# Dsouza10082/nats-llm-studio

Measured on AMD Instinct MI355X. Metric: output tokens/sec + p50 NATS req-reply RTT, Llama-3-8B Q4_K chat_model, higher is better.
Workload: dtype fp16; 1 GPU; model=llama-3-8b Q4_K_M, global_batch=512, seq_len=128, parallelism=dp1, concurrency_per_replica=512, hipgraph=True, device=cuda

## Files before the change

### csrc/kernels/qgemv.hip

```cpp
#include "qgemm_impl.h"
#include "qgemm_dma.h"

using namespace nls_gemv;

namespace nls_hgemm {
int launch_dense(int wm, int bn, int waves, int nst, const SegList& sl, int ntiles, int ks, float* ws,
                 const GemvArgs& a, hipStream_t st);
}
namespace nls_hg10 {
int launch_dense10(int bn, const SegList& sl, int ntiles, int ks, float* ws, const GemvArgs& a, hipStream_t st);
}
namespace nls_q9 {
int launch_q9(int kset, int waves, int rt, const SegList& sl, int ntiles, int ks, float* ws, const GemvArgs& a,
              hipStream_t st, int bm);
}


extern "C" {

struct NlsSeg {
  const void* w;
  const int* xmap;
  const int* ymap;
  const int* mcount;
  int type, rows, K, ycol;
};

struct NlsFuse {
  const float* xf; long ldxf; const float* nw; float eps;
  const int* pos; const int* slot; const float* cs; const float* bias;
  void* q_out; long ldq; void* kc; void* vc; int Hq, Hkv, D, pad0;
  void* hout; long ldh; const float* onw; int* cnt;
  float* ssq_out; const float* ssq_in; int ldss, nss_in;
  const int* sel; int sel_slots, sel_base, pad1;
  const void* wr; int E, topk, renorm, rcap;
  float* rlogits; float* topw; int* counts; int* xrows; int* yrows; int* rsel;
  const void* tab; int tab_n, tab_cap;
};

struct NlsPlan {
  int kset;
  int tile_rows;
  int tiles;
  int cols;
  int slab_width;
  int mapped_splitk;
  int reduce;
  int pad;
  long ws_floats;
};

}

namespace {

inline bool mapped(const NlsSeg& s) { return s.xmap || s.ymap || s.mcount; }

bool norm_in_ok(const NlsFuse& f, int M, int mode) {
  if (f.xf && (M > 16 || !f.nw || (mode != 0 && !(mode == 1 && f.ssq_in)))) return false;
  if (f.ssq_in && (!f.xf || f.nss_in < 1 || f.nss_in > f.ldss)) return false;
  return true;
}

bool norm_producer_ok(const NlsFuse& f, const NlsSeg* segs, int nseg, int M, int epi, const void* argmax, int waves,
                      int rt, int mode) {
  if (!f.ssq_out) return true;
  const int ncols = ((M + 15) / 16) * 16;
  return !(mode != 0 || epi != EPI_ADD_F32 || nseg != 1 || mapped(segs[0]) || argmax || f.onw || M > 32 ||
           (waves * 64) % ncols || f.ldss < (segs[0].rows + 16 * rt - 1) / (16 * rt));
}

bool rope_ok(const NlsFuse& f, const NlsSeg* segs, int nseg, int epi, const void* argmax, int mode, int ks) {
  if (epi != EPI_ROPE) return true;
  if (!(mode == 0 || ((mode == 4 || mode == 5 || mode == 10) && ks <= 1)) || argmax || !f.pos || !f.slot || !f.cs ||
      !f.q_out || !f.kc || !f.vc || f.D < 2 || f.D % 2 || f.Hq < 1 || f.Hkv < 1)
    return false;
  int c = 0;
  for (int i = 0; i < nseg; ++i) {
    if (mapped(segs[i]) || segs[i].rows % 16 || segs[i].ycol != c) return false;
    c += segs[i].rows;
  }
  return c == (f.Hq + 2 * f.Hkv) * f.D;
}

bool add_norm_ok(const NlsFuse& f, const NlsSeg* segs, int nseg, int M, int epi, const void* argmax, int mode) {
  if (f.onw && (mode != 0 || epi != EPI_ADD_F32 || nseg != 1 || segs[0].ycol || mapped(segs[0]) || !f.cnt ||
                !f.hout || segs[0].rows % 4 || argmax))
    return false;
  if (f.wr && (!f.onw || M > 4 || f.E < 1 || f.E > 64 || f.topk < 1 || f.topk > f.E || f.topk > 8 || !f.rlogits ||
               !f.topw || !f.counts || !f.xrows || !f.yrows || segs[0].rows % 4))
    return false;
  return true;
}

bool selected_ok(const NlsFuse& f, const NlsSeg* segs, int nseg, const void* argmax, int mode) {
  if (!f.sel) return true;
  if (mode != 0 || f.sel_slots < 1 || f.sel_slots > 256 || argmax) return false;
  for (int i = 1; i < nseg; ++i)
    if (segs[i].rows != segs[0].rows || segs[i].K != segs[0].K) return false;
  return true;
}

bool table_ok(const NlsFuse& f, const NlsSeg* segs, int nseg, int epi, const void* argmax, int mode, int ks) {
  if (!f.tab) return true;
  return !(nseg != 1 || mode < 0 || mode > 2 || ks > 1 || f.tab_n < 1 || f.tab_cap < 1 || !segs[0].mcount ||
           argmax || f.xf || f.onw || f.ssq_out || epi == EPI_ROPE || epi == EPI_SLABS);
}

bool mode_shape_ok(const NlsFuse& f, const NlsSeg* segs, int nseg, long ldx, long ldy, int M, int epi, int waves,
                   int rt, int mode) {
  if (waves != 4 && waves != 8 && !(waves == 16 && mode >= 4) && !(waves == 7 && mode == 1 && rt == 1 && M == 1))
    return false;
  if (mode < 0 || mode > 10 || mode == 7 || mode == 8 || (mode == 6 && (waves != 8 || rt != 2))) return false;
  const bool unaligned_y = (epi == EPI_F32 || epi == EPI_ADD_F32 || epi == EPI_ACT) && ldy % 4;
  if (mode == 10) {
    if (waves != 8 || (rt != 1 && rt != 2) || f.xf || f.onw || ldx % 8 || unaligned_y) return false;
    for (int i = 0; i < nseg; ++i)
      if (segs[i].type != QT_F16 || mapped(segs[i]) || segs[i].ycol % 4) return false;
  } else if (mode == 9) {
    if (!((waves == 4 && rt == 2) || (waves == 8 && (rt == 2 || rt == 1))) || f.xf || f.onw || epi == EPI_ROPE ||
        ldx % 8 || unaligned_y)
      return false;
    for (int i = 0; i < nseg; ++i)
      if (mapped(segs[i]) || segs[i].ycol % 4) return false;
  } else if (mode >= 4) {
    if ((waves != 8 && waves != 16) || (rt != 2 && rt != 4) || f.xf || f.onw || (epi == EPI_ROPE && mode == 6))
      return false;
    for (int i = 0; i < nseg; ++i)
      if (segs[i].type != QT_F16) return false;
  } else if (mode == 3) {
    if (waves != 4 || (rt != 4 && rt != 6 && rt != 8 && rt != 16)) return false;
    for (int i = 0; i < nseg; ++i)
      if (segs[i].type == QT_Q8_0) return false;
  } else if (mode == 2 ? (waves != 8 || (rt != 1 && rt != 2 && rt != 4)) : (rt != 1 && rt != 2)) {
    return false;
  }
  return !(M > 64 && mode == 0);
}

int type_set(const NlsSeg* segs, int nseg) {
  bool q4k = false, q5k = false, q6k = false, q8 = false, q51 = false, iq4 = false, flt = false, bad = false;
  for (int i = 0; i < nseg; ++i) {
    const int t = segs[i].type;
    if (t == QT_Q4_K) q4k = true;
    else if (t == QT_Q5_K) q5k = true;
    else if (t == QT_Q8_0) q8 = true;
    else if (t == QT_Q51) q51 = true;
    else if (t == QT_IQ4) iq4 = true;
    else if (t == QT_F16 || t == QT_BF16 || t == QT_F32) flt = true;
    else if (t == QT_Q6_K) q6k = true;
    else bad = true;
  }
  if (bad || (flt && (q4k || q5k || q6k || q8 || q51 || iq4)) || (q4k && (q5k || q8 || q51 || iq4)) ||
      (q51 && (q5k || iq4)))
    return -1;
  return flt ? 2 : (q51 ? 3 : (iq4 ? 4 : (q4k ? 0 : ((q5k || q8) ? 1 : 0))));
}

inline int mtiles(int M) { return M > 64 ? 8 : (M + 15) / 16; }
inline int mblocks(int M) { return M > 64 ? (M + 127) / 128 : 1; }

int plan(const NlsSeg* segs, int nseg, const void* x, long ldx, void* y, long ldy, int M, float alpha, int epi,
         void* argmax, int waves, int rt, int mode, int ks, const void* ws, long ws_floats, const NlsFuse& f,
         NlsPlan& p, SegList& sl, GemvArgs& a) {
  if (nseg < 1 || nseg > 8 || M < 1) return -1;
  if (!mode_shape_ok(f, segs, nseg, ldx, ldy, M, epi, waves, rt, mode) || !norm_in_ok(f, M, mode) ||
      !norm_producer_ok(f, segs, nseg, M, epi, argmax, waves, rt, mode) ||
      !rope_ok(f, segs, nseg, epi, argmax, mode, ks) || !add_norm_ok(f, segs, nseg, M, epi, argmax, mode) ||
      !selected_ok(f, segs, nseg, argmax, mode) || !table_ok(f, segs, nseg, epi, argmax, mode, ks))
    return -1;
  if (mode != 0 && ks > 1 && !ws) return -1;
  if (epi == EPI_SLABS && (mode == 0 || ks < 2)) return -1;
  bool mks = (mode >= 1 && mode <= 5) && ks > 1 && epi == EPI_F32 && !argmax;
  for (int i = 0; i < nseg && mks; ++i)
    mks = segs[i].ymap && segs[i].ycol == 0 && segs[i].rows == segs[0].rows;
  sl = SegList{};
  int tiles = 0, cols = 0;
  const int tile_rows = mode == 10 ? 256 / rt : mode == 9 ? 16 * waves * rt
                        : (mode == 5 ? 256 : (mode >= 2 ? 128 : (mode == 1 ? waves : 1) * rt * 16));
  for (int i = 0; i < nseg; ++i) {
    if (segs[i].K % 256 || segs[i].rows < 1) return -1;
    if (epi == EPI_SWIGLU && segs[i].rows % 16) return -1;
    if (mapped(segs[i]) && mode != 0 &&
        (!(mode >= 1 && mode <= 5) || argmax || epi == EPI_SLABS || (ks > 1 && !mks)))
      return -1;
    sl.s[i] = Seg{(const uint8_t*)segs[i].w, segs[i].xmap, segs[i].ymap, segs[i].mcount, segs[i].type, segs[i].rows,
                  segs[i].K,  tiles, segs[i].ycol,  cols};
    tiles += (segs[i].rows + tile_rows - 1) / tile_rows;
    cols += segs[i].rows;
  }
  sl.nseg = nseg;
  if (f.tab) tiles *= f.tab_n;
  const int sel_tiles = (segs[0].rows + tile_rows - 1) / tile_rows;
  if (f.sel) tiles = f.sel_slots * sel_tiles;
  const int kset = type_set(segs, nseg);
  if (kset < 0) return -1;
  if (mode >= 2 && mode <= 3 && kset >= 2) return -1;
  if (mode == 9 && kset == 2) return -1;
  const int nks = mode != 0 && ks > 1 ? ks : 1;
  if (mode == 0 && f.xf && !staged_lds_a(sl, waves, rt, mtiles(M), M)) return -1;
  if (mode == 1 && (f.xf || waves == 7) && !staged_lds_b(sl, mtiles(M), M, nks, mblocks(M), f.xf)) return -1;
  p = NlsPlan{};
  p.kset = kset;
  p.tile_rows = tile_rows;
  p.tiles = tiles;
  p.cols = cols;
  p.slab_width = mks ? segs[0].rows : cols;
  p.mapped_splitk = mks;
  p.reduce = nks > 1 && epi != EPI_SLABS;
  p.ws_floats = nks > 1 ? (long)nks * M * p.slab_width : 0;
  if (ws_floats < p.ws_floats) return -1;
  a = GemvArgs{(const act_t*)(f.xf ? (const void*)f.xf : x), ldx, y, ldy, M, epi, alpha,  p.slab_width,
               (unsigned long long*)argmax,  0,  M,
               f.xf, f.ldxf, f.nw, f.eps,
               f.pos, f.slot, f.cs, f.bias, (__bf16*)f.q_out, f.ldq, (__bf16*)f.kc, (__bf16*)f.vc, f.Hq, f.Hkv, f.D,
               (act_t*)f.hout, f.ldh, f.onw, f.cnt,
               f.ssq_out, f.ssq_in, f.ldss, f.nss_in,
               f.sel, sel_tiles, f.sel_base,  0,
               (const act_t*)f.wr, f.E, f.topk, f.renorm, f.rcap,
               f.rlogits, f.topw, f.counts, f.xrows, f.yrows, f.rsel,
               (const uint8_t* const*)f.tab, f.tab_n, f.tab_cap};
  return 0;
}

int run(const NlsPlan& p, const SegList& sl, const GemvArgs& a, int waves, int rt, int mode, int ks, float* ws,
        hipStream_t st) {
  const int M = a.M, mt = mtiles(M);
  auto launch = p.kset == 0 ? launch_k0
                            : p.kset == 1 ? launch_k1 : p.kset == 2 ? launch_k2 : p.kset == 3 ? launch_k3 : launch_k4;
  if (mode == 0) return launch(0, waves, rt, mt, sl, p.tiles, 1, nullptr, a, st, 1);
  if (ks < 1) ks = 1;
  int rc;
  if (mode == 10)
    rc = nls_hg10::launch_dense10(256 / rt, sl, p.tiles, ks, ws, a, st);
  else if (mode == 9)
    rc = nls_q9::launch_q9(p.kset, waves, rt, sl, p.tiles, ks, ws, a, st, 256);
  else if (mode >= 4)
    rc = nls_hgemm::launch_dense(rt, mode == 5 ? 256 : 128, waves, mode == 6 ? 2 : 3, sl, p.tiles, ks, ws, a, st);
  else if (mode == 3)
    rc = (p.kset == 0 ? nls_dma::launch_dma_k0 : nls_dma::launch_dma_k1)(rt, sl, p.tiles, ks, ws, a, st);
  else if (mode == 2)
    rc = (p.kset == 0 ? nls_gemm::launch_lds_k0 : nls_gemm::launch_lds_k1)(rt, sl, p.tiles, ks, ws, a, st);
  else
    rc = launch(1, waves, rt, mt, sl, p.tiles, ks, ws, a, st, mblocks(M));
  if (rc || !p.reduce) return rc;
  RedList rl{};
  if (p.mapped_splitk) {
    rl.s[0] = RedSeg{0, p.slab_width, 0, 0};
    rl.nseg = 1;
  } else {
    for (int i = 0; i < sl.nseg; ++i) rl.s[i] = RedSeg{sl.s[i].tile_begin_col, sl.s[i].rows, sl.s[i].ycol, 0};
    rl.nseg = sl.nseg;
  }
  const int nout = a.epi == EPI_SWIGLU ? p.slab_width / 2 : p.slab_width;
  dim3 grid((nout + 255) / 256, M);
  hipLaunchKernelGGL(splitk_reduce_kernel, grid, dim3(256), 0, st, (const float*)ws, ks, M, p.slab_width, rl, a);
  return (int)hipGetLastError();
}

const NlsFuse kNoFuse{};

}

extern "C" {

int nls_qgemv(const NlsSeg* segs, int nseg, const void* x, long ldx, void* y, long ldy, int M, float alpha, int epi,
              void* argmax, int waves, int rt, int mode, int ks, void* ws, long ws_floats, void* stream,
              const NlsFuse* fz) {
  NlsPlan p;
  SegList sl;
  GemvArgs a;
  if (plan(segs, nseg, x, ldx, y, ldy, M, alpha, epi, argmax, waves, rt, mode, ks, ws, ws_floats, fz ? *fz : kNoFuse,
           p, sl, a))
    return -1;
  return run(p, sl, a, waves, rt, mode, ks, (float*)ws, (hipStream_t)stream);
}

int nls_qgemv_plan(const NlsSeg* segs, int nseg, const void* x, long ldx, void* y, long ldy, int M, float alpha,
                   int epi, void* argmax, int waves, int rt, int mode, int ks, void* ws, long ws_floats, void* stream,
                   const NlsFuse* fz, NlsPlan* out) {
  SegList sl;
  GemvArgs a;
  (void)stream;
  return plan(segs, nseg, x, ldx, y, ldy, M, alpha, epi, argmax, waves, rt, mode, ks, ws, ws_floats,
              fz ? *fz : kNoFuse, *out, sl, a);
}

int nls_fuse_size() { return (int)sizeof(NlsFuse); }
int nls_plan_size() { return (int)sizeof(NlsPlan); }

}
```

### nats_llm_studio_amd/ops/__init__.py

```python
from __future__ import annotations

import ctypes
import math
import warnings
from dataclasses import dataclass
from typing import List, Optional, Sequence

import numpy as np
import torch

from ..gguf.constants import GGMLType, GGML_BLOCK
from ..gguf.quants import dequantize
from . import _lib
from . import transcode

EPI = {"f32": 0, "act": 1, "add": 2, "swiglu": 3, "slabs": 4, "argmax": 5, "rope": 6}
import os as _os
ADDNORM_MAX_M = int(_os.environ.get("NLS_ADDNORM", "0"))
DENSE_MIN_M = int(_os.environ.get("NLS_DENSE_GEMM_M", "128"))
MOE_GEMV = tuple(int(v) for v in _os.environ.get("NLS_MOE_GEMV", "0,4,2,1").split(","))
ACT_DTYPE = torch.float16


def _stream_ptr(t: torch.Tensor) -> int:
# ... 72 lines not shown
class QWeight:

    def __init__(self, raw: np.ndarray, ggml_type: int, rows: int, K: int, device, name: str = "",
                 layout: str = "tiled"):
        self.gtype = int(ggml_type)
        self.type = int(ggml_type)
        self.rows = int(rows)
        self.K = int(K)
        self.name = name
        self.layout = layout
        self.device = torch.device(device)
        if K % 256:
            raise ValueError(f"{name}: K={K} is not a multiple of 256")
        with warnings.catch_warnings():
            warnings.simplefilter("ignore", UserWarning)
            if GGMLType(ggml_type) in transcode.TRANSCODED:
                t = torch.from_numpy(np.ascontiguousarray(np.asarray(raw).view(np.uint8).reshape(-1)))
                t = t.to(self.device) if self.device.type != "cpu" else t
                t, self.type = transcode.device_form(t, ggml_type, rows, K, layout)
                if layout == "rows":
                    t = torch.from_numpy(np.ascontiguousarray(to_device_layout(t.cpu().numpy(), self.type, rows, K)))
                    self.data = t.to(self.device) if self.device.type != "cpu" else t.clone()
                elif self.type in (transcode.QT_Q51, transcode.QT_IQ4):
                    self.data = t
                else:
                    self.data = tile_layout(t, self.type, rows, K)
            elif layout == "rows":
                t = torch.from_numpy(np.ascontiguousarray(to_device_layout(raw, ggml_type, rows, K)))
                self.data = t.to(self.device) if self.device.type != "cpu" else t.clone()
            else:
                t = torch.from_numpy(np.ascontiguousarray(np.asarray(raw).view(np.uint8).reshape(-1)))
                t = t.to(self.device) if self.device.type != "cpu" else t
                self.data = tile_layout(t, ggml_type, rows, K)
        self._raw = np.ascontiguousarray(raw).view(np.uint8).reshape(-1) if self.device.type == "cpu" else None
        self._dense = None
        self.d16: Optional[torch.Tensor] = None

    def to_f16(self) -> "QWeight":
        if self.device.type == "cpu" or self.type == int(GGMLType.F16):
            return self
        w = QWeight.__new__(QWeight)
        w.__dict__.update(self.__dict__)
        w.type = int(GGMLType.F16)
        w.data = tile_layout(self.dense(torch.float16).contiguous().view(torch.uint8).reshape(-1), GGMLType.F16,
                             self.rows, self.K)
        w.d16 = None
        return w

    def expand_dense(self) -> int:
        if self.device.type != "cuda" or self.layout != "tiled" or self.d16 is not None:
            return 0
        self.d16 = self.dense(torch.float16).contiguous()
        return self.d16.numel() * 2

    @staticmethod
    def expand_dense_group(ws: Sequence["QWeight"]) -> int:
        ws = list(ws)
        if (len(ws) < 2 or any(w.device.type != "cuda" or w.layout != "tiled" or w.d16 is not None for w in ws)
                or len({w.K for w in ws}) != 1 or len({str(w.device) for w in ws}) != 1):
            return sum(w.expand_dense() for w in ws)
        buf = torch.empty(sum(w.rows for w in ws), ws[0].K, dtype=torch.float16, device=ws[0].device)
        r0 = 0
        for w in ws:
            buf[r0:r0 + w.rows].copy_(w.dense(torch.float16))
            w.d16 = buf[r0:r0 + w.rows]
            r0 += w.rows
        return buf.numel() * 2

    @property
    def dense_bytes(self) -> int:
        return self.rows * self.K * 2

    @property
    def nbytes(self) -> int:
        return self.data.numel()

    def dense(self, dtype=torch.float32) -> torch.Tensor:
        if self.device.type == "cpu":
            if self._dense is None:
                self._dense = torch.from_numpy(dequantize(self._raw, self.gtype, (self.rows, self.K)).copy())
            return self._dense.to(dtype)
        out = torch.empty(self.rows, self.K, dtype=ACT_DTYPE, device=self.device)
        _lib.check(_lib.lib().nls_dequant(self.data.data_ptr(), self.type, self.rows, self.K, out.data_ptr(),
                                          self.K, _stream_ptr(out)), "nls_dequant")
        return out.to(dtype)


def kernel_set(types) -> Optional[int]:
    ts = set(int(t) for t in types)
    flt = ts & {0, 1, 30}
    q4k, q5k, q8, q51, iq4 = 12 in ts, 13 in ts, 8 in ts, transcode.QT_Q51 in ts, transcode.QT_IQ4 in ts
    if ts - {0, 1, 30, 8, 12, 13, 14, transcode.QT_Q51, transcode.QT_IQ4}:
        return None
    if (flt and ts - flt) or (q4k and (q5k or q8 or q51 or iq4)) or (q51 and (q5k or iq4)):
        return None
    return 2 if flt else (3 if q51 else (4 if iq4 else (0 if q4k else (1 if (q5k or q8) else 0))))


def interleave_gate_up(gate_raw: np.ndarray, up_raw: np.ndarray, ggml_type: int, rows: int, K: int,
                       group: int = 8) -> np.ndarray:
    rb = row_bytes(ggml_type, K)
    g = np.asarray(gate_raw).view(np.uint8).reshape(rows // group, group, rb)
    u = np.asarray(up_raw).view(np.uint8).reshape(rows // group, group, rb)
    return np.ascontiguousarray(np.concatenate([g, u], axis=1)).reshape(-1)


@dataclass
class Seg:
    w: QWeight
    ycol: int = 0
    xmap: Optional[torch.Tensor] = None
    ymap: Optional[torch.Tensor] = None
    mcount: Optional[torch.Tensor] = None


class ExpertTable:

    def __init__(self, ws: Sequence[QWeight]):
        self.ws = list(ws)
        w0 = self.ws[0]
        if any((w.type, w.rows, w.K, w.layout, w.device) != (w0.type, w0.rows, w0.K, w0.layout, w0.device)
               for w in self.ws):
            raise ValueError("ExpertTable: the experts of a projection must share type, shape and device")
        self.ptrs = None
        if w0.device.type == "cuda":
            self.ptrs = torch.tensor([w.data.data_ptr() for w in self.ws], dtype=torch.int64, device=w0.device)

    def __len__(self) -> int:
        return len(self.ws)


_WS = {}
_WS_OLD = []


def _workspace(dev, n: int) -> torch.Tensor:
    w = _WS.get(dev)
    if w is None or w.numel() < n:
        if w is not None:
            _WS_OLD.append(w)
        w = torch.empty(max(n, 16 << 20), dtype=torch.float32, device=dev)
        _WS[dev] = w
    return w


def dense_ok(segs: Sequence[Seg], M: int) -> bool:
    return M >= DENSE_MIN_M and all(s.w.d16 is not None and s.xmap is None and s.ymap is None for s in segs)


def gemv_config(segs: Sequence[Seg], M: int):
    from . import tuning
    if dense_ok(segs, M):
        cfg = tuning.select_dense(segs, M)
        if cfg is not None:
            return cfg
    return tuning.select(segs, M)


DENSE_MODES = (4, 5, 6, 10)


def _merge_dense(segs: Sequence[Seg]):
    out = []
    for s in segs:
        if s.w.d16 is None:
            raise ValueError(f"{s.w.name}: dense modes {DENSE_MODES} need QWeight.expand_dense()")
        p = s.w.d16.data_ptr()
        plain = s.xmap is None and s.ymap is None and s.mcount is None
        if out and plain and out[-1][4].xmap is None and out[-1][4].ymap is None and out[-1][4].mcount is None:
            q, rows, K, ycol, s0 = out[-1]
            if K == s.w.K and q + rows * K * 2 == p and ycol + rows == s.ycol:
                out[-1] = [q, rows + s.w.rows, K, ycol, s0]
                continue
        out.append([p, s.w.rows, s.w.K, s.ycol, s])
    return out


def _seg_arr(segs: Sequence[Seg], mode: int):
    if mode in DENSE_MODES:
        merged = _merge_dense(segs)
        arr = (_lib.NlsSeg * len(merged))()
        for i, (p, rows, K, ycol, s) in enumerate(merged):
            arr[i] = _lib.NlsSeg(p, _p(s.xmap), _p(s.ymap), _p(s.mcount), 1, rows, K, ycol)
        return arr
    arr = (_lib.NlsSeg * len(segs))()
    for i, s in enumerate(segs):
        arr[i] = _lib.NlsSeg(s.w.data.data_ptr(), _p(s.xmap), _p(s.ymap), _p(s.mcount), s.w.type, s.w.rows, s.w.K,
                             s.ycol)
    return arr


NORM_FUSE_LDS = 54 * 1024


def norm_fusable(M: int, K: int) -> bool:
    return M <= 16 and M * K * 2 <= NORM_FUSE_LDS


def _ws_floats(segs: Sequence[Seg], M: int, mode: int, ks: int) -> int:
    if mode == 0 or ks <= 1:
        return 0
    return ks * M * (segs[0].w.rows if all(s.ymap is not None for s in segs) else sum(s.w.rows for s in segs))


def _launch(segs: Sequence[Seg], x: torch.Tensor, y: torch.Tensor, M: int, alpha: float, epi: str, cfg, *, fz=None,
            argmax: Optional[torch.Tensor] = None, label: str = "nls_qgemv", soft: bool = False) -> bool:
    mode, waves, rt, ks = cfg
    arr = _seg_arr(segs, mode)
    n = _ws_floats(segs, M, mode, ks)
    ws = _workspace(x.device, n).data_ptr() if n else None
    rc = _lib.lib().nls_qgemv(arr, len(arr), x.data_ptr(), x.stride(0), y.data_ptr(), y.stride(0), M, float(alpha),
                              EPI[epi], _p(argmax), waves, rt, mode, ks, ws, n, _stream_ptr(x),
                              None if fz is None else ctypes.byref(fz))
    if soft and rc == -1:
        return False
    _lib.check(rc, label)
    return True


def _launch_slabs(segs: Sequence[Seg], x: torch.Tensor, y: torch.Tensor, M: int, alpha: float, cfg) -> torch.Tensor:
    _launch(segs, x, y, M, alpha, "slabs", cfg)
    return _WS[x.device]


def _fuse_norm(norm) -> "_lib.NlsFuse":
    xf, nw, eps = norm[:3]
    fz = _lib.NlsFuse(xf=xf.data_ptr(), ldxf=xf.stride(0), nw=nw.data_ptr(), eps=float(eps))
    if len(norm) == 6 and norm[3] is not None:
        fz.ssq_in, fz.ldss, fz.nss_in = norm[3].data_ptr(), int(norm[4]), int(norm[5])
    return fz


def _fuse_rope(fz, pos, slot, cs, bias, q_out, kc, vc, Hq: int, Hkv: int, D: int):
    fz.pos, fz.slot, fz.cs, fz.bias = pos.data_ptr(), slot.data_ptr(), cs.data_ptr(), _p(bias)
    fz.q_out, fz.ldq, fz.kc, fz.vc = q_out.data_ptr(), q_out.stride(0), kc.data_ptr(), vc.data_ptr()
    fz.Hq, fz.Hkv, fz.D = Hq, Hkv, D
    return fz


def _check_table(segs: Sequence[Seg], table, norm, argmax):
    tab, cap = table
    s0 = segs[0]
    if len(segs) != 1 or s0.mcount is None or s0.w is not tab.ws[0] or norm is not None or argmax is not None:
        raise ValueError("qgemv(table=): one mapped segment over the table's first expert")
    if s0.mcount.numel() < len(tab) or any(t is not None and t.numel() < len(tab) * cap for t in (s0.xmap, s0.ymap)):
        raise ValueError("qgemv(table=): row maps / counts shorter than the table's experts x cap")


def qgemv(segs: Sequence[Seg], x: torch.Tensor, y: torch.Tensor, M: int, alpha: float = 1.0, epi: str = "f32",
          argmax: Optional[torch.Tensor] = None, waves: int = 0, rt: int = 1, mode: int = -1, ks: int = 1,
          norm=None, sel=None, table=None):
    if not x.is_cuda:
        return _qgemv_cpu(segs, x, y, M, alpha, epi, argmax, norm, table)
    mapped = any(s.xmap is not None for s in segs)
    if norm is not None:
        return _qgemv_norm(segs, y, M, alpha, epi, argmax, norm, mapped)
    if table is not None:
        _check_table(segs, table, norm, argmax)
    if x.dtype != ACT_DTYPE:
        raise TypeError(f"qgemv: activations must be {ACT_DTYPE}, got {x.dtype}")
    routed = sel is not None or table is not None
    if not mapped and not routed and (x.shape[0] < M or (epi != "argmax" and y.shape[0] < M)):
        raise ValueError(f"qgemv: M={M} rows but x has {x.shape[0]}, y {y.shape[0]}")
    if mode < 0 or waves == 0:
        mode, waves, rt, ks = MOE_GEMV if mapped or routed else gemv_config(segs, M)
    if sel is not None:
        mode, ks = 0, (1 if table is None else ks)
    if M > 64 and mode == 0 and not routed:
        for m0 in range(0, M, 64):
            mm = min(64, M - m0)
            qgemv(segs, x[m0:], y[m0:], mm, alpha, epi, None if argmax is None else argmax[m0:], waves, rt,
                  mode, ks)
        return y
    fz, label = None, "nls_qgemv"
    if routed:
        fz, label = _lib.NlsFuse(), "nls_qgemv(sel)"
        if sel is not None:
            fz.sel, fz.sel_slots, fz.sel_base = sel[0].data_ptr(), int(sel[1]), int(sel[2])
        if table is not None:
            fz.tab, fz.tab_n, fz.tab_cap = table[0].ptrs.data_ptr(), len(table[0]), int(table[1])
            label = "nls_qgemv(table)"
    _launch(segs, x, y, M, alpha, epi, (mode, waves, rt, ks), fz=fz, argmax=argmax, label=label)
    return y


def _qgemv_norm(segs, y, M, alpha, epi, argmax, norm, mapped):
    split = len(norm) == 6 and norm[3] is not None
    if split and (mapped or M > 16):
        raise ValueError("fused-norm GEMV needs unmapped rows and M <= 16")
    if not split and (mapped or not norm_fusable(M, segs[0].w.K)):
        raise ValueError("fused-norm GEMV needs unmapped rows and M*K*2 <= NORM_FUSE_LDS")
    cfg = gemv_config(segs, M)
    if split:
        cands, label = ([cfg] if cfg[0] in (0, 1) else []) + [(0, 4, 2, 1)], "nls_qgemv(norm+ssq)"
    else:
        cands, label = [(0, cfg[1], cfg[2], 1) if cfg[0] == 0 else (0, 4, 2, 1)], "nls_qgemv(norm)"
    fz = _fuse_norm(norm)
    for c in cands:
        if _launch(segs, norm[0], y, M, alpha, epi, c, fz=fz, argmax=argmax, label=label, soft=split):
            return y
    raise ValueError("no launch config takes the split-RMSNorm operands")


def _qgemv_cpu(segs, x, y, M, alpha, epi, argmax, norm, table):
    if norm is not None:
        xf, nw, eps = norm[:3]
        xs = xf[:M].float()
        x = (xs * torch.rsqrt(xs.pow(2).mean(dim=1, keepdim=True) + eps) * nw.float()).to(ACT_DTYPE)
    if table is not None:
        _check_table(segs, table, norm, argmax)
        (tab, cap), s0 = table, segs[0]
        segs = [Seg(w, s0.ycol, None if s0.xmap is None else s0.xmap[e * cap:],
# ... 98 lines not shown
        keys.fill_(torch.iinfo(torch.int64).min)



def rmsnorm(x: torch.Tensor, w: torch.Tensor, out: torch.Tensor, M: int, eps: float):
    D = x.shape[1]
    if x.is_cuda:
        _lib.check(_lib.lib().nls_rmsnorm(x.data_ptr(), x.stride(0), w.data_ptr(), out.data_ptr(), out.stride(0), M,
                                          D, float(eps), int(out.dtype == torch.float32), _stream_ptr(x)),
                   "nls_rmsnorm")
        return out
    xs = x[:M].float()
    r = xs * torch.rsqrt(xs.pow(2).mean(dim=1, keepdim=True) + eps) * w.float()
    out[:M] = r.to(out.dtype)
    return out


def rope_inv_freq(head_dim: int, base: float, freq_factors=None) -> np.ndarray:
    inv = 1.0 / (base ** (np.arange(0, head_dim, 2, dtype=np.float64) / head_dim))
    if freq_factors is not None:
        inv = inv / np.asarray(freq_factors, dtype=np.float64).reshape(-1)[:head_dim // 2]
    return inv


def rope_table(max_pos: int, head_dim: int, base: float, device, freq_factors=None,
               pos_scale: float = 1.0) -> torch.Tensor:
    inv = rope_inv_freq(head_dim, base, freq_factors)
    ang = (np.arange(max_pos, dtype=np.float64) * pos_scale)[:, None] * inv[None, :]
    cs = np.stack([np.cos(ang), np.sin(ang)], axis=-1).astype(np.float32)
    return torch.from_numpy(cs).to(device)


KV_DTYPES = {"bf16": torch.bfloat16, "fp8": torch.float8_e4m3fn}


def _kv_fn(name: str, kc: torch.Tensor):
    if kc.dtype == torch.float8_e4m3fn:
        return getattr(_lib.lib(), name + "8")
    if kc.dtype != torch.bfloat16:
        raise TypeError(f"{name}: KV cache dtype {kc.dtype} (bf16 or float8_e4m3fn)")
    return getattr(_lib.lib(), name)


def _kv_cast(v: torch.Tensor, dtype) -> torch.Tensor:
    if dtype == torch.float8_e4m3fn:
        v = v.clamp(-448.0, 448.0)
    return v.to(dtype)


def rope_kv(qkv: torch.Tensor, pos: torch.Tensor, slot: torch.Tensor, cs: torch.Tensor, q_out: torch.Tensor,
            kc: torch.Tensor, vc: torch.Tensor, T: int, Hq: int, Hkv: int, D: int, neox: bool = False,
            bias: Optional[torch.Tensor] = None):
    if qkv.is_cuda:
        _lib.check(_kv_fn("nls_rope_kv", kc)(qkv.data_ptr(), qkv.stride(0), 1, 0, _p(bias), pos.data_ptr(),
                                          slot.data_ptr(), cs.data_ptr(), q_out.data_ptr(), q_out.stride(0),
                                          kc.data_ptr(), vc.data_ptr(), T, Hq, Hkv, D, int(neox), _stream_ptr(qkv)),
                   "nls_rope_kv")
        return
    x = qkv[:T, :(Hq + 2 * Hkv) * D].float()
    if bias is not None:
        x = x + bias.float()[None, :x.shape[1]]
    p = pos[:T].long()
    c, s = cs[p, :, 0], cs[p, :, 1]

    def rot(h):
        if neox:
            x0, x1 = h[..., :D // 2], h[..., D // 2:]
        else:
            x0, x1 = h[..., 0::2], h[..., 1::2]
        cc, ss = c[:, None, :], s[:, None, :]
        y0, y1 = x0 * cc - x1 * ss, x0 * ss + x1 * cc
        if neox:
            return torch.cat([y0, y1], dim=-1)
        return torch.stack([y0, y1], dim=-1).flatten(-2)

    q = rot(x[:, :Hq * D].view(T, Hq, D))
    k = rot(x[:, Hq * D:(Hq + Hkv) * D].view(T, Hkv, D))
    v = x[:, (Hq + Hkv) * D:(Hq + 2 * Hkv) * D].view(T, Hkv, D)
    q_out[:T, :Hq * D] = q.reshape(T, Hq * D).to(q_out.dtype)
    sl = slot[:T].long()
    ok = sl >= 0
    kc[sl[ok]] = _kv_cast(k[ok], kc.dtype)
    vc[sl[ok]] = _kv_cast(v[ok], vc.dtype)


def qk_norm_rope_kv(qkv: torch.Tensor, pos: torch.Tensor, slot: torch.Tensor, cs: torch.Tensor, q_out: torch.Tensor,
                    kc: torch.Tensor, vc: torch.Tensor, T: int, Hq: int, Hkv: int, D: int, qw: torch.Tensor,
                    kw: torch.Tensor, eps: float, neox: bool = False, ks: int = 1, slab: int = 0):
    if qkv.is_cuda:
        if qw.dtype != torch.float32 or kw.dtype != torch.float32 or qw.numel() != D or kw.numel() != D:
            raise ValueError(f"qk_norm_rope_kv: norm weights must be f32 [{D}]")
        _lib.check(_kv_fn("nls_qknorm_rope_kv", kc)(qkv.data_ptr(), qkv.stride(0), int(ks), int(slab), qw.data_ptr(),
                                                    kw.data_ptr(), float(eps), pos.data_ptr(), slot.data_ptr(),
                                                    cs.data_ptr(), q_out.data_ptr(), q_out.stride(0), kc.data_ptr(),
                                                    vc.data_ptr(), T, Hq, Hkv, D, int(neox), _stream_ptr(qkv)),
                   "nls_qknorm_rope_kv")
        return
    ncol = (Hq + 2 * Hkv) * D
    ld = qkv.stride(0)
    flat = qkv.reshape(-1).float()
    x = torch.zeros(T, ncol)
    for k in range(ks):
        x = x + torch.as_strided(flat, (T, ncol), (ld, 1), k * slab)
    p = pos[:T].long()
    c, s = cs[p, :, 0], cs[p, :, 1]

    def rms(h, w):
        return h * torch.rsqrt(h.pow(2).mean(-1, keepdim=True) + eps) * w.float()

    def rot(h):
        if neox:
            x0, x1 = h[..., :D // 2], h[..., D // 2:]
        else:
            x0, x1 = h[..., 0::2], h[..., 1::2]
        cc, ss = c[:, None, :], s[:, None, :]
        y0, y1 = x0 * cc - x1 * ss, x0 * ss + x1 * cc
        if neox:
            return torch.cat([y0, y1], dim=-1)
        return torch.stack([y0, y1], dim=-1).flatten(-2)

    q = rot(rms(x[:, :Hq * D].view(T, Hq, D), qw))
    k = rot(rms(x[:, Hq * D:(Hq + Hkv) * D].view(T, Hkv, D), kw))
    v = x[:, (Hq + Hkv) * D:].view(T, Hkv, D)
    q_out[:T, :Hq * D] = q.reshape(T, Hq * D).to(q_out.dtype)
    sl = slot[:T].long()
    ok = sl >= 0
    kc[sl[ok]] = _kv_cast(k[ok], kc.dtype)
    vc[sl[ok]] = _kv_cast(v[ok], vc.dtype)


def qkv_rope_kv(segs: Sequence[Seg], h: torch.Tensor, qkv: torch.Tensor, pos: torch.Tensor, slot: torch.Tensor,
                cs: torch.Tensor, q_out: torch.Tensor, kc: torch.Tensor, vc: torch.Tensor, T: int, Hq: int, Hkv: int,
                D: int, neox: bool = False, cfg=None, bias: Optional[torch.Tensor] = None, norm=None,
                fuse_rope: bool = True, qk_norm=None):
    if qk_norm is not None and bias is not None:
        raise ValueError("qkv_rope_kv: a Q/K norm with a QKV bias is not supported")

    def rope(src, ks=1, slab=0):
        if qk_norm is not None:
            return qk_norm_rope_kv(src, pos, slot, cs, q_out, kc, vc, T, Hq, Hkv, D, *qk_norm, neox, ks=ks, slab=slab)
        if ks == 1:
            return rope_kv(src, pos, slot, cs, q_out, kc, vc, T, Hq, Hkv, D, neox, bias)
        _lib.check(_kv_fn("nls_rope_kv", kc)(src.data_ptr(), src.stride(0), ks, slab, _p(bias), pos.data_ptr(),
                                             slot.data_ptr(), cs.data_ptr(), q_out.data_ptr(), q_out.stride(0),
                                             kc.data_ptr(), vc.data_ptr(), T, Hq, Hkv, D, int(neox), _stream_ptr(h)),
                   "nls_rope_kv")

    if h.is_cuda and all(s.xmap is None for s in segs):
        mode, waves, rt, ks = cfg or gemv_config(segs, T)
        ncol = sum(s.w.rows for s in segs)
        plain = (ncol == (Hq + 2 * Hkv) * D
                 and all(s.ycol == sum(x.w.rows for x in segs[:i]) for i, s in enumerate(segs)))
        epilogue = plain and qk_norm is None and not neox and fuse_rope and kc.dtype == torch.bfloat16
        if epilogue and ((mode == 0 and T <= 64) or (mode in (4, 5, 10) and ks == 1 and norm is None)):
            if norm is not None and not norm_fusable(T, segs[0].w.K):
                raise ValueError("fused-norm GEMV needs M*K*2 <= NORM_FUSE_LDS")
            fz = _fuse_rope(_lib.NlsFuse() if norm is None else _fuse_norm(norm), pos, slot, cs, bias, q_out, kc, vc,
                            Hq, Hkv, D)
            _launch(segs, h, qkv, T, 1.0, "rope", (mode, waves, rt, 1), fz=fz,
                    label="nls_qgemv(rope)" if mode == 0 else "nls_qgemv(dense rope)")
            return
        if norm is None and mode != 0 and ks > 1 and plain:
            ws = _launch_slabs(segs, h, qkv, T, 1.0, (mode, waves, rt, ks))
            return rope(ws[:ks * T * ncol].view(ks * T, ncol), ks, T * ncol)
        if norm is None and cfg is not None and qk_norm is not None:
            qgemv(segs, h, qkv, T, waves=waves, rt=rt, mode=mode, ks=ks)
            return rope(qkv)
    qgemv(segs, h, qkv, T, norm=norm)
    rope(qkv)


def embed(ids: torch.Tensor, w: QWeight, out: torch.Tensor, T: int, scale: float = 1.0, prev=None):
    if ids.is_cuda:
        if prev is not None:
            nxt, use = prev
            _lib.check(_lib.lib().nls_embed_prev(ids.data_ptr(), nxt.data_ptr(), use.data_ptr(), T, w.data.data_ptr(),
                                                 w.type, w.rows, w.K, out.data_ptr(), out.stride(0), float(scale),
                                                 _stream_ptr(ids)), "nls_embed_prev")
            return out
        _lib.check(_lib.lib().nls_embed(ids.data_ptr(), T, w.data.data_ptr(), w.type, w.rows, w.K, out.data_ptr(),
                                        out.stride(0), float(scale), _stream_ptr(ids)), "nls_embed")
        return out
    if prev is not None:
        nxt, use = prev
        torch.where(use[:T] != 0, nxt[:T], ids[:T], out=ids[:T])
    out[:T] = scale * w.dense()[ids[:T].long()]
    return out


def attention(q: torch.Tensor, kc: torch.Tensor, vc: torch.Tensor, block_tables: torch.Tensor,
              tok_seq: torch.Tensor, ctx_len: torch.Tensor, out: torch.Tensor, T: int, Hq: int, Hkv: int, D: int,
              block_size: int, scale: float, chunk: int = 256, n_split: int = 1,
              workspace: Optional[torch.Tensor] = None, counters: Optional[torch.Tensor] = None):
    if q.is_cuda:
        po = pml = None
        if counters is not None and (counters.numel() < T * Hkv or counters.dtype != torch.int32):
            raise ValueError("attention counters must be int32 with >= T*Hkv entries")
        if n_split > 1:
            need = T * Hq * n_split * (D + 2)
            if workspace is None or workspace.numel() < need:
                workspace = torch.empty(need, dtype=torch.float32, device=q.device)
            po = workspace.data_ptr()
            pml = po + T * Hq * n_split * D * 4
        _lib.check(_kv_fn("nls_attn_decode", kc)(q.data_ptr(), q.stride(0), kc.data_ptr(), vc.data_ptr(),
                                              block_tables.data_ptr(), block_tables.stride(0), tok_seq.data_ptr(),
                                              ctx_len.data_ptr(), T, Hq, Hkv, D, block_size, float(scale), chunk,
                                              n_split, out.data_ptr(), out.stride(0), po, pml,
                                              _p(counters) if n_split > 1 else None, _stream_ptr(q)),
                   "nls_attn_decode")
        return out
    G = Hq // Hkv
    for t in range(T):
        n = int(ctx_len[t])
        if n <= 0:
            out[t, :Hq * D] = 0
            continue
        bt = block_tables[int(tok_seq[t])].long()
        p = torch.arange(n)
        slots = bt[p // block_size] * block_size + p % block_size
        k = kc[slots].float()
        v = vc[slots].float()
        qq = q[t, :Hq * D].float().view(Hkv, G, D)
        s = torch.einsum("hgd,nhd->hgn", qq, k) * scale
        pr = torch.softmax(s, dim=-1)
        o = torch.einsum("hgn,nhd->hgd", pr, v)
        out[t, :Hq * D] = o.reshape(Hq * D).to(out.dtype)
    return out


PREFILL_V1 = _os.environ.get("NLS_PREFILL_V1", "0") == "1"
PREFILL_QT = 32 if PREFILL_V1 else 64


def prefill_blocks(tok_seq, pos, T: int):
    ts = np.asarray(tok_seq[:T])
    ps = np.asarray(pos[:T])
    if T == 0:
        return np.zeros((0, 4), np.int32)
    cut = np.flatnonzero((ts[1:] != ts[:-1]) | (ps[1:] != ps[:-1] + 1)) + 1
    starts = np.concatenate([[0], cut])
    ends = np.concatenate([cut, [T]])
    out = []
    for a, b in zip(starts, ends):
        for t in range(a, b, PREFILL_QT):
            out.append((t, min(PREFILL_QT, b - t), ts[a], ps[t]))
    return np.asarray(out, dtype=np.int32).reshape(-1, 4)


def attention_prefill_ok(Hq: int, Hkv: int, D: int) -> bool:
    return Hq % Hkv == 0 and (Hq // Hkv) % 4 == 0 and D in (64, 128)


def attention_prefill(q: torch.Tensor, kc: torch.Tensor, vc: torch.Tensor, block_tables: torch.Tensor,
                      qblocks: torch.Tensor, nqb: int, tok_seq: torch.Tensor, ctx_len: torch.Tensor,
                      out: torch.Tensor, T: int, Hq: int, Hkv: int, D: int, block_size: int, scale: float):
    if q.is_cuda:
        _lib.check(_kv_fn("nls_attn_prefill_v1" if PREFILL_V1 else "nls_attn_prefill", kc)(q.data_ptr(), q.stride(0), kc.data_ptr(), vc.data_ptr(),
                                               block_tables.data_ptr(), block_tables.stride(0), qblocks.data_ptr(),
                                               nqb, Hq, Hkv, D, block_size, float(scale), out.data_ptr(),
                                               out.stride(0), _stream_ptr(q)), "nls_attn_prefill")
        return out
    return attention(q, kc, vc, block_tables, tok_seq, ctx_len, out, T, Hq, Hkv, D, block_size, scale)


def argmax(logits: torch.Tensor, M: int, out: torch.Tensor):
    V = logits.shape[1]
    if logits.is_cuda:
        _lib.check(_lib.lib().nls_argmax(logits.data_ptr(), logits.stride(0), M, V, out.data_ptr(),
                                         _stream_ptr(logits)), "nls_argmax")
        return out
    out[:M] = logits[:M].float().argmax(dim=1).to(out.dtype)
    return out


def topc_candidates(logits: torch.Tensor, n: int, C: int, vocab_lo: int, valid: int):
    if logits.is_cuda:
        if logits.dtype != torch.float32 or logits.stride(1) != 1:
            raise TypeError("topc_candidates: fp32 row-major logits")
        src = torch.empty(2, n, C, dtype=torch.int32, device=logits.device)
        _lib.check(_lib.lib().nls_topc(logits.data_ptr(), logits.stride(0), n, int(valid), C, int(vocab_lo),
                                       src.data_ptr(), _stream_ptr(logits)), "nls_topc")
        v, i = src[0].view(torch.float32), src[1]
        v._packed = i._packed = src
        return v, i
    k = max(0, min(C, valid))
    v = torch.full((n, C), float("-inf"), dtype=torch.float32, device=logits.device)
    i = torch.full((n, C), -1, dtype=torch.int32, device=logits.device)
    if k and n:
        tv, ti = torch.topk(logits[:n, :valid].float(), k, dim=1)
        ti, order = torch.sort(ti, dim=1)
        v[:, :k] = torch.gather(tv, 1, order)
        i[:, :k] = (ti + vocab_lo).to(torch.int32)
    return v, i


def argmax_unpack(keys: torch.Tensor, n: int, out: torch.Tensor, rearm: bool = False):
    if keys.is_cuda:
        fn = _lib.lib().nls_argmax_unpack_rearm if rearm else _lib.lib().nls_argmax_unpack
        _lib.check(fn(keys.data_ptr(), n, out.data_ptr(), _stream_ptr(keys)), "nls_argmax_unpack")
        return out
    out[:n] = (0xFFFFFFFF - (keys[:n] & 0xFFFFFFFF)).to(out.dtype)
    if rearm:
        argmax_reset(keys[:n])
    return out


SAMPLE_PARAMS_BYTES = 40
# ... 341 lines not shown
```

Baseline: 41850 output tokens/s.

## Add 128x96 MFMA dense GEMM kernel mode 14 with 4-stage LDS DMA pipeline

Adds a new dense fp16 GEMM kernel (mode 14) using 128x96 block tiles, 8 waves, a 4-slot global-to-LDS DMA ring with swizzled reads and prioritized MFMA, plus fused RoPE/KV-cache epilogue. It wires the mode into planning, validation and the Python dispatcher, and falls back to mode 4 when segments cannot merge. Whether it is used depends on the tuning table selecting mode 14, which is not shown here. The aim is better tile utilization for prefill-size M. The cost is more complex barrier choreography and a split-K parity constraint.

```diff
diff --git a/csrc/kernels/hgemm14.hip b/csrc/kernels/hgemm14.hip
--- /dev/null
+++ b/csrc/kernels/hgemm14.hip
@@ -0,0 +1,264 @@
+#include "qgemm_dma.h"
+
+namespace nls_hg14 {
+using namespace nls_gemv;
+using nls_dma::glds16;
+using nls_dma::lds_addr;
+
+constexpr int BM = 128, BN = 96;
+constexpr int UB = 128 * 128;
+constexpr int SLOT = 2 * UB;
+constexpr int R = 4;
+constexpr int MTW = 2, NTW = BN / 32;
+
+template <int N>
+DEVI void wait_vm() {
+  asm volatile("s_waitcnt vmcnt(%0)" ::"i"(N) : "memory");
+}
+
+DEVI void h14_rope(const f32x4 (&acc)[MTW][NTW], const Seg& S, int rbase, int mbase, const GemvArgs& a) {
+  const int lane = threadIdx.x & 63;
+  const int r = lane & 15, g = lane >> 4;
+  const int M = a.M, D = a.D;
+  const bool odd = r & 1;
+  int col[NTW], hd[NTW], dd[NTW];
+  float b0[NTW], b1[NTW];
+  bool okr[NTW];
+#pragma unroll
+  for (int j = 0; j < NTW; ++j) {
+    const int row = rbase + 16 * j + r;
+    okr[j] = row < S.rows;
+    col[j] = S.ycol + row;
+    hd[j] = col[j] / D;
+    dd[j] = col[j] - hd[j] * D;
+    b0[j] = a.bias && okr[j] ? a.bias[col[j] & ~1] : 0.f;
+    b1[j] = a.bias && okr[j] ? a.bias[col[j] | 1] : 0.f;
+  }
+#pragma unroll
+  for (int i = 0; i < MTW; ++i) {
+    long slot[4];
+    const float* csr[4];
+    bool okb[4];
+    float2 c[4][NTW];
+#pragma unroll
+    for (int e = 0; e < 4; ++e) {
+      const int b = mbase + 16 * i + 4 * g + e;
+      okb[e] = b < M;
+      const int bg = a.m0 + (okb[e] ? b : 0);
+      slot[e] = a.slot[bg];
+      csr[e] = a.cs + (size_t)a.pos[bg] * D;
+    }
+#pragma unroll
+    for (int e = 0; e < 4; ++e)
+#pragma unroll
+      for (int j = 0; j < NTW; ++j)
+        c[e][j] = hd[j] < a.Hq + a.Hkv ? reinterpret_cast<const float2*>(csr[e])[dd[j] >> 1] : float2{1.f, 0.f};
+#pragma unroll
+    for (int e = 0; e < 4; ++e) {
+      const int b = a.m0 + mbase + 16 * i + 4 * g + e;
+#pragma unroll
+      for (int j = 0; j < NTW; ++j) {
+        const float v = acc[i][j][e] * a.alpha;
+        const float p = __shfl_xor(v, 1, 64);
+        float x0 = odd ? p : v, x1 = odd ? v : p;
+        if (a.bias) {
+          x0 += b0[j];
+          x1 += b1[j];
+        }
+        const int h = hd[j];
+        const long s = slot[e];
+        float y = odd ? x1 : x0;
+        __bf16* d = nullptr;
+        if (h < a.Hq + a.Hkv) {
+          const float2 cc = c[e][j];
+          y = odd ? x0 * cc.y + x1 * cc.x : x0 * cc.x - x1 * cc.y;
+          if (h < a.Hq) d = a.q_out + (size_t)b * a.ldq + col[j];
+          else if (s >= 0) d = a.kc + ((size_t)s * a.Hkv + (h - a.Hq)) * D + dd[j];
+        } else if (s >= 0) {
+          d = a.vc + ((size_t)s * a.Hkv + (h - a.Hq - a.Hkv)) * D + dd[j];
+        }
+        if (d && okb[e] && okr[j]) *d = (__bf16)y;
+      }
+    }
+  }
+}
+
+DEVI void h14_epilogue(const f32x4 (&acc)[MTW][NTW], const Seg& S, int row0, int kslice, int ks, const GemvArgs& a,
+                       float* ws) {
+  const int lane = threadIdx.x & 63;
+  const int wave = __builtin_amdgcn_readfirstlane(threadIdx.x >> 6);
+  const int r = lane & 15, g = lane >> 4;
+  const int M = a.M;
+  const int rbase = row0 + (wave >> 2) * (BN / 2), mbase = (wave & 3) * 32;
+  if (ks > 1) {
+    const int ntot = a.pad;
+#pragma unroll
+    for (int j = 0; j < NTW; ++j) {
+      const int row = rbase + 16 * j + r;
+      if (row >= S.rows) continue;
+#pragma unroll
+      for (int i = 0; i < MTW; ++i)
+#pragma unroll
+        for (int e = 0; e < 4; ++e) {
+          const int b = mbase + 16 * i + 4 * g + e;
+          if (b >= M) continue;
+          ws[((size_t)kslice * a.mtot + a.m0 + b) * ntot + S.tile_begin_col + row] = acc[i][j][e];
+        }
+    }
+    return;
+  }
+  if (a.epi == EPI_ROPE) {
+    h14_rope(acc, S, rbase, mbase, a);
+    return;
+  }
+#pragma unroll
+  for (int j = 0; j < NTW; ++j) {
+    const int row = rbase + 16 * j + r;
+#pragma unroll
+    for (int i = 0; i < MTW; ++i) {
+#pragma unroll
+      for (int e = 0; e < 4; ++e) {
+        const int b = mbase + 16 * i + 4 * g + e;
+        const float v = acc[i][j][e] * a.alpha;
+        if (b < M && row < S.rows) {
+          const size_t off = (size_t)b * a.ldy + S.ycol + row;
+          if (a.epi == EPI_F32) reinterpret_cast<float*>(a.y)[off] = v;
+          else if (a.epi == EPI_ADD_F32) reinterpret_cast<float*>(a.y)[off] += v;
+          else if (a.epi == EPI_ACT) reinterpret_cast<act_t*>(a.y)[off] = (act_t)v;
+        }
+      }
+    }
+  }
+}
+
+DEVI void h14_tile(const Seg& S, int row0, int kslice, int ks, const GemvArgs& a, float* ws, uint8_t* lds) {
+  const int lane = threadIdx.x & 63;
+  const int wave = __builtin_amdgcn_readfirstlane(threadIdx.x >> 6);
+  const int wr = wave >> 2, wc = wave & 3;
+  const int r = lane & 15, g = lane >> 4;
+  const int nk64 = S.K >> 6;
+  const int p0 = (nk64 * kslice) / ks;
+  const int np = (nk64 * (kslice + 1)) / ks - p0;
+  const int M = a.M;
+
+  const int c = (lane & 7) ^ (lane >> 3);
+  const bool wone = wr == 1;
+  const int wg0 = wone ? 8 + (wave & 3) : 2 * wave;
+  const act_t* Wd = reinterpret_cast<const act_t*>(S.w);
+  const act_t* xsrc[2];
+  const act_t* wsrc[2];
+#pragma unroll
+  for (int i = 0; i < 2; ++i) {
+    const int xr = 8 * (2 * wave + i) + (lane >> 3);
+    xsrc[i] = a.x + (size_t)min(xr, M - 1) * a.ldx + p0 * 64 + c * 8;
+    const int wrow = min(8 * (wg0 + i) + (lane >> 3), BN - 1);
+    wsrc[i] = Wd + (size_t)min(row0 + wrow, S.rows - 1) * S.K + p0 * 64 + c * 8;
+  }
+  const uint32_t base = __builtin_amdgcn_readfirstlane(lds_addr(lds));
+  const uint32_t xdst = base + (uint32_t)(2 * wave) * 1024u, wdst = base + UB + (uint32_t)wg0 * 1024u;
+  auto dma = [&](int q, int slot) __attribute__((always_inline)) {
+    const int koff = min(q, np - 1) * 64;
+    const uint32_t so = (uint32_t)slot * SLOT;
+    glds16(xsrc[0] + koff, xdst + so);
+    glds16(xsrc[1] + koff, xdst + so + 1024);
+    glds16(wsrc[0] + koff, wdst + so);
+    if (!wone) glds16(wsrc[1] + koff, wdst + so + 1024);
+  };
+  auto wait_pairs = [&](auto n) __attribute__((always_inline)) {
+    constexpr int N = decltype(n)::value;
+    if (wone) wait_vm<3 * N>();
+    else wait_vm<4 * N>();
+  };
+
+  f16x8 A[MTW], B[NTW];
+  const int xo = (wc * 32 + r) * 128, wo = UB + (wr * (BN / 2) + r) * 128;
+  auto rd = [&](int slot, int t) __attribute__((always_inline)) {
+    const uint8_t* sb = lds + slot * SLOT;
+    const int co = ((4 * t + g) ^ (r & 7)) << 4;
+#pragma unroll
+    for (int i = 0; i < MTW; ++i) A[i] = *reinterpret_cast<const f16x8*>(sb + xo + i * 2048 + co);
+#pragma unroll
+    for (int j = 0; j < NTW; ++j) B[j] = *reinterpret_cast<const f16x8*>(sb + wo + j * 2048 + co);
+  };
+  f32x4 acc[MTW][NTW];
+#pragma unroll
+  for (int i = 0; i < MTW; ++i)
+#pragma unroll
+    for (int j = 0; j < NTW; ++j) acc[i][j] = f32x4{0.f, 0.f, 0.f, 0.f};
+  auto mma = [&]() __attribute__((always_inline)) {
+    asm volatile("s_waitcnt lgkmcnt(0)" ::: "memory");
+    __builtin_amdgcn_s_setprio(1);
+#pragma unroll
+    for (int i = 0; i < MTW; ++i)
+#pragma unroll
+      for (int j = 0; j < NTW; ++j) acc[i][j] = mfma16(A[i], B[j], acc[i][j]);
+    __builtin_amdgcn_s_setprio(0);
+  };
+  auto bar = []() __attribute__((always_inline)) {
+    __builtin_amdgcn_s_barrier();
+    asm volatile("" ::: "memory");
+  };
+
+  if (np > 0) {
+#pragma unroll
+    for (int q = 0; q < R - 1; ++q) dma(q, q);
+    wait_pairs(std::integral_constant<int, R - 2>{});
+    bar();
+    if (wr == 1) bar();
+    int slot = 0, prev = R - 1;
+    for (int s = 0; s < np; ++s) {
+      rd(slot, 0);
+      bar();
+      mma();
+      wait_pairs(std::integral_constant<int, R - 3>{});
+      bar();
+      rd(slot, 1);
+      dma(s + R - 1, prev);
+      bar();
+      mma();
+      bar();
+      prev = slot;
+      slot = slot + 1 == R ? 0 : slot + 1;
+    }
+    if (wr == 0) bar();
+  }
+  wait_vm<0>();
+
+  h14_epilogue(acc, S, row0, kslice, ks, a, ws);
+}
+
+__global__ __launch_bounds__(512, 1) void hgemm14_kernel(SegList segs, GemvArgs a, int ks, float* ws, int ntiles,
+                                                          int nmb) {
+  extern __shared__ __attribute__((aligned(16))) uint8_t h14lds[];
+  const nls_dma::GridPos gp = nls_dma::dense_grid_pos(blockIdx.x, ks, nmb, 0);
+  const int kslice = gp.kslice, mb = gp.mb, tile = gp.tile;
+  if (tile >= ntiles) return;
+  const int m0 = mb * BM;
+  Seg S = segs.s[0];
+#pragma unroll
+  for (int s = 1; s < 8; ++s)
+    if (s < segs.nseg && tile >= segs.s[s].tile_begin) S = segs.s[s];
+  a.m0 = m0;
+  a.x += (size_t)m0 * a.ldx;
+  const size_t esz = (a.epi == EPI_F32 || a.epi == EPI_ADD_F32) ? 4 : 2;
+  a.y = (char*)a.y + (size_t)m0 * a.ldy * esz;
+  a.M = min(BM, a.M - m0);
+  h14_tile(S, (tile - S.tile_begin) * BN, kslice, ks, a, ws, h14lds);
+}
+
+int launch_dense14(const SegList& sl, int ntiles, int ks, float* ws, const GemvArgs& a, hipStream_t st) {
+  constexpr int LDS = R * SLOT;
+  const int nmb = (a.M + BM - 1) / BM;
+  const int grid = nls_dma::dense_grid(ntiles, nmb, ks, 0);
+  static bool attr = false;
+  if (!attr) {
+    const hipError_t e = hipFuncSetAttribute((const void*)hgemm14_kernel, hipFuncAttributeMaxDynamicSharedMemorySize,
+                                             LDS);
+    if (e != hipSuccess) return (int)e;
+    attr = true;
+  }
+  hipLaunchKernelGGL(hgemm14_kernel, dim3(grid), dim3(512), LDS, st, sl, a, ks, ws, ntiles, nmb);
+  return (int)hipGetLastError();
+}
+
+}
diff --git a/csrc/kernels/qgemv.hip b/csrc/kernels/qgemv.hip
--- a/csrc/kernels/qgemv.hip
+++ b/csrc/kernels/qgemv.hip
@@ -9,6 +9,9 @@
 }
 namespace nls_hg10 {
 int launch_dense10(int bn, const SegList& sl, int ntiles, int ks, float* ws, const GemvArgs& a, hipStream_t st);
+}
+namespace nls_hg14 {
+int launch_dense14(const SegList& sl, int ntiles, int ks, float* ws, const GemvArgs& a, hipStream_t st);
 }
 namespace nls_q9 {
 int launch_q9(int kset, int waves, int rt, const SegList& sl, int ntiles, int ks, float* ws, const GemvArgs& a,
@@ -72,8 +75,9 @@
 
 bool rope_ok(const NlsFuse& f, const NlsSeg* segs, int nseg, int epi, const void* argmax, int mode, int ks) {
   if (epi != EPI_ROPE) return true;
-  if (!(mode == 0 || ((mode == 4 || mode == 5 || mode == 10) && ks <= 1)) || argmax || !f.pos || !f.slot || !f.cs ||
-      !f.q_out || !f.kc || !f.vc || f.D < 2 || f.D % 2 || f.Hq < 1 || f.Hkv < 1)
+  const bool dense = mode == 4 || mode == 5 || mode == 10 || mode == 14;
+  if (!(mode == 0 || (dense && ks <= 1)) || argmax || !f.pos || !f.slot || !f.cs || !f.q_out || !f.kc || !f.vc ||
+      f.D < 2 || f.D % 2 || f.Hq < 1 || f.Hkv < 1)
     return false;
   int c = 0;
   for (int i = 0; i < nseg; ++i) {
@@ -111,9 +115,15 @@
                    int rt, int mode) {
   if (waves != 4 && waves != 8 && !(waves == 16 && mode >= 4) && !(waves == 7 && mode == 1 && rt == 1 && M == 1))
     return false;
-  if (mode < 0 || mode > 10 || mode == 7 || mode == 8 || (mode == 6 && (waves != 8 || rt != 2))) return false;
+  if (mode < 0 || (mode > 10 && mode != 14) || mode == 7 || mode == 8 || (mode == 6 && (waves != 8 || rt != 2)))
+    return false;
   const bool unaligned_y = (epi == EPI_F32 || epi == EPI_ADD_F32 || epi == EPI_ACT) && ldy % 4;
-  if (mode == 10) {
+  if (mode == 14) {
+    if (waves != 8 || rt != 2 || f.xf || f.onw || ldx % 8 || unaligned_y) return false;
+    if (epi == EPI_SWIGLU || epi == EPI_ARGMAX) return false;
+    for (int i = 0; i < nseg; ++i)
+      if (segs[i].type != QT_F16 || mapped(segs[i]) || segs[i].ycol % 4) return false;
+  } else if (mode == 10) {
     if (waves != 8 || (rt != 1 && rt != 2) || f.xf || f.onw || ldx % 8 || unaligned_y) return false;
     for (int i = 0; i < nseg; ++i)
       if (segs[i].type != QT_F16 || mapped(segs[i]) || segs[i].ycol % 4) return false;
@@ -170,17 +180,20 @@
       !selected_ok(f, segs, nseg, argmax, mode) || !table_ok(f, segs, nseg, epi, argmax, mode, ks))
     return -1;
   if (mode != 0 && ks > 1 && !ws) return -1;
+  if (mode == 14 && argmax) return -1;
   if (epi == EPI_SLABS && (mode == 0 || ks < 2)) return -1;
   bool mks = (mode >= 1 && mode <= 5) && ks > 1 && epi == EPI_F32 && !argmax;
   for (int i = 0; i < nseg && mks; ++i)
     mks = segs[i].ymap && segs[i].ycol == 0 && segs[i].rows == segs[0].rows;
   sl = SegList{};
   int tiles = 0, cols = 0;
-  const int tile_rows = mode == 10 ? 256 / rt : mode == 9 ? 16 * waves * rt
+  const int tile_rows = mode == 14 ? 96 : mode == 10 ? 256 / rt : mode == 9 ? 16 * waves * rt
                         : (mode == 5 ? 256 : (mode >= 2 ? 128 : (mode == 1 ? waves : 1) * rt * 16));
   for (int i = 0; i < nseg; ++i) {
     if (segs[i].K % 256 || segs[i].rows < 1) return -1;
     if (epi == EPI_SWIGLU && segs[i].rows % 16) return -1;
+    for (int s = 1; mode == 14 && s < ks; ++s)
+      if (((segs[i].K / 64) * s / ks) % 2) return -1;
     if (mapped(segs[i]) && mode != 0 &&
         (!(mode >= 1 && mode <= 5) || argmax || epi == EPI_SLABS || (ks > 1 && !mks)))
       return -1;
@@ -231,7 +244,9 @@
   if (mode == 0) return launch(0, waves, rt, mt, sl, p.tiles, 1, nullptr, a, st, 1);
   if (ks < 1) ks = 1;
   int rc;
-  if (mode == 10)
+  if (mode == 14)
+    rc = nls_hg14::launch_dense14(sl, p.tiles, ks, ws, a, st);
+  else if (mode == 10)
     rc = nls_hg10::launch_dense10(256 / rt, sl, p.tiles, ks, ws, a, st);
   else if (mode == 9)
     rc = nls_q9::launch_q9(p.kset, waves, rt, sl, p.tiles, ks, ws, a, st, 256);
diff --git a/nats_llm_studio_amd/ops/__init__.py b/nats_llm_studio_amd/ops/__init__.py
--- a/nats_llm_studio_amd/ops/__init__.py
+++ b/nats_llm_studio_amd/ops/__init__.py
@@ -248,12 +248,14 @@
     from . import tuning
     if dense_ok(segs, M):
         cfg = tuning.select_dense(segs, M)
+        if cfg is not None and cfg[0] == 14 and len(_merge_dense(segs)) > 1:
+            cfg = (4, 16, 2, cfg[3])
         if cfg is not None:
             return cfg
     return tuning.select(segs, M)
 
 
-DENSE_MODES = (4, 5, 6, 10)
+DENSE_MODES = (4, 5, 6, 10, 14)
 
 
 def _merge_dense(segs: Sequence[Seg]):
@@ -658,7 +660,7 @@
         plain = (ncol == (Hq + 2 * Hkv) * D
                  and all(s.ycol == sum(x.w.rows for x in segs[:i]) for i, s in enumerate(segs)))
         epilogue = plain and qk_norm is None and not neox and fuse_rope and kc.dtype == torch.bfloat16
-        if epilogue and ((mode == 0 and T <= 64) or (mode in (4, 5, 10) and ks == 1 and norm is None)):
+        if epilogue and ((mode == 0 and T <= 64) or (mode in (4, 5, 10, 14) and ks == 1 and norm is None)):
             if norm is not None and not norm_fusable(T, segs[0].w.K):
                 raise ValueError("fused-norm GEMV needs M*K*2 <= NORM_FUSE_LDS")
             fz = _fuse_rope(_lib.NlsFuse() if norm is None else _fuse_norm(norm), pos, slot, cs, bias, q_out, kc, vc,
```

Result: faster. 42300 output tokens/s (median of 6 runs) (+1.1%).
